# loryruta/gl-radix-sort

Measured on AMD Instinct MI355X. Metric: Mkeys/s sorting 2^28 uint32 key+val; % HBM roofline; 1/2/4/8 GPU, higher is better.
Workload: dtype u32; 1 GPU; 2^28 uint32 key + uint32 val pairs, uniform-random full-range keys, vals=iota, in-place stable radix sort, 1x MI355X; pairs_per_gpu=268435456, key_distribution=uniform, parallelism=single, device=AMD Radeon Graphics (gfx950:sramecc+:xnack-), 256 CUs, 288.0 GiB, device 0

## Files before the change

gl-radix-sort_amd/csrc/glu_hip.hip:

```cpp
#include <hip/hip_runtime.h>

#include <algorithm>
#include <cstdio>
#include <cstdlib>
#include <cstring>
#include <mutex>
#include <strings.h>
#include <vector>

#include "glu_host.hpp"
#include "glu_sort_driver.hpp"
#include "glu_sort_launch.hpp"
#include "radix_sort_kernels.hpp"
#include "radix_pair_passes.hpp"
#include "radix_lds_plan.hpp"

using namespace glu_hip;
using namespace glu_hip::host;

glu_status glu_hip::host::sort_prepare(glu_radix_sort_s* s, size_t count, size_t key_size, bool with_vals, bool may_place)
{
    if (count <= 1) return GLU_OK;
    const bool grows = s->keys.size < count * key_size || (with_vals && s->vals.size < count * sizeof(uint32_t));
    if (grows && !s->tuning)
// ... 208 lines not shown
    int cur = 0;
    uint32_t pass = 0;
    for (; pass < num_passes; pass++)
    {
        const uint32_t shift = passes[pass].shift, bits = passes[pass].bits, xform = passes[pass].xform;
        if (planned)
        {
            PlanArgs pa;
            pa.plan = (PassPlan*) s->plan.ptr;
            pa.pass = pass;
            pa.may_skip = xform == 0;
            if (key_xf == KEY_XF_NONE && !s->no_bit_shortcut) pa.flags = pass == 0 ? kPlanCollectBits : (pa.may_skip ? kPlanShortcut : 0u);
            pa.pair_role = passes[pass].pair_role;
            if (pa.pair_role == 1)
            {
                pa.shift2 = passes[pass + 1].shift;
                pa.bits2 = passes[pass + 1].bits;
            }
            s->cur_kind = finish_kpt && pass < 2 ? 1 : 0;
            pa.behind_attempt = finish_kpt && pass >= 2;
            s->cur_behind = pa.behind_attempt;
            if (finish_kpt && pass == 0)
            {
                pa.finish_geo_first = finish_kpt;
                pa.finish_geo_last = finish_last;
                pa.finish_first_ordinary = 2;
                pa.finish_num_ordinary = num_passes - 2;
                pa.finish_seq = s->feedback.finish_seq;
                pa.finish_top_bit = finish_top_bit;
                pa.finish_key_bits = end_bit;
                pa.finish_long_ok = finish_long_ok;
                pa.fork_side = fork;
            }
            pa.unitsum_side = fork && pass == 1 && pa.pair_role == 2 && bits == 8;
            if (finish_kpt && pass < 2 && s->last_narrow_offered) pa.narrow_keys = narrow_keys;
            GLU_TRY(dispatch_pass<KeyT>(s, kbuf[0], vbuf[0], kbuf[1], vbuf[1], count, shift, bits, nullptr,
                                        fork && pa.behind_attempt ? s->side : stream, xform, pa));
            if (finish_kpt && pass == 1)
            {
                if (fork) HIP_TRY(hipEventRecord(s->ev_fork2, stream));
                s->cur_kind = 2;
                s->cur_behind = false;
                s->mark(stream);
                s->mark(stream);
                const FinishMarks finish_marks{[](void* object, hipStream_t st) { ((glu_radix_sort_s*) object)->mark(st, true); }, s};
                const auto finish = vals ? (key_xf != KEY_XF_NONE ? launch_finish<KeyT, true, true> : launch_finish<KeyT, true, false>)
                                         : (key_xf != KEY_XF_NONE ? launch_finish<KeyT, false, true> : launch_finish<KeyT, false, false>);
                GLU_TRY(finish(kbuf[0], vbuf[0], kbuf[1], vbuf[1], (const uint32_t*) s->finish_starts.ptr, finish_kpt, finish_last, finish_expected,
                               finish_top_bit - 16u, pa.plan, 2u, key_xf, stream, s->finish_rank_bits, (uint32_t*) s->finish_crowded.ptr, finish_marks,
                               s->last_narrow_offered ? (const uint16_t*) narrow_keys : (const uint16_t*) nullptr));
                if (finish_long_ok && !fork)
                    GLU_TRY(launch_long_run_passes_any<KeyT>(s, kbuf[0], vbuf[0], kbuf[1], vbuf[1], count, key_xf, stream));
            }
        }
        else
        {
            GLU_TRY(dispatch_pass<KeyT>(s, kbuf[cur], vbuf[cur], kbuf[cur ^ 1], vbuf[cur ^ 1], count, shift, bits, nullptr,
                                        stream, xform));
            cur ^= 1;
        }
    }
    s->cur_behind = false;
    if (fork)
    {
        HIP_TRY(hipStreamWaitEvent(s->side, s->ev_fork2, 0));
        if (finish_long_ok) GLU_TRY(launch_long_run_passes_any<KeyT>(s, kbuf[0], vbuf[0], kbuf[1], vbuf[1], count, key_xf, s->side));
        HIP_TRY(side_join.join());
    }
    if (planned)
    {
        const dim3 grid((uint32_t) std::min<size_t>((count + 255) / 256, (size_t) g_dev.num_cus * 16));
        const auto finalize = vals ? radix_finalize_kernel<KeyT, true> : radix_finalize_kernel<KeyT, false>;
        hipLaunchKernelGGL(finalize, grid, dim3(256), 0, stream, kbuf[0], vbuf[0], (const KeyT*) kbuf[1], (const uint32_t*) vbuf[1],
                           (uint32_t) count, (const PassPlan*) s->plan.ptr, pass, finish_kpt ? 2u : 0u);
        HIP_TRY(hipGetLastError());
        return GLU_OK;
    }
    if (cur == 1)
    {
        HIP_TRY(hipMemcpyAsync(keys, kbuf[1], count * sizeof(KeyT), hipMemcpyDeviceToDevice, stream));
        if (vals) HIP_TRY(hipMemcpyAsync(vals, vbuf[1], count * sizeof(uint32_t), hipMemcpyDeviceToDevice, stream));
    }
    return GLU_OK;
}

template<typename KeyT>
glu_status glu_hip::host::sort_run(glu_radix_sort_s* s, KeyT* keys, uint32_t* vals, size_t count, size_t num_steps, hipStream_t stream,
                                   uint32_t key_xf)
{
    constexpr size_t kMaxSteps = sizeof(KeyT) * 2;
    const size_t steps = (num_steps == 0 || num_steps > kMaxSteps) ? kMaxSteps : num_steps;
    return sort_bits<KeyT>(s, keys, vals, count, 0u, (uint32_t) steps * 4, stream, key_xf);
}
template glu_status glu_hip::host::sort_bits<uint32_t>(glu_radix_sort_s*, uint32_t*, uint32_t*, size_t, uint32_t, uint32_t, hipStream_t, uint32_t);
template glu_status glu_hip::host::sort_bits<uint64_t>(glu_radix_sort_s*, uint64_t*, uint32_t*, size_t, uint32_t, uint32_t, hipStream_t, uint32_t);
template glu_status glu_hip::host::sort_run<uint32_t>(glu_radix_sort_s*, uint32_t*, uint32_t*, size_t, size_t, hipStream_t, uint32_t);
template glu_status glu_hip::host::sort_run<uint64_t>(glu_radix_sort_s*, uint64_t*, uint32_t*, size_t, size_t, hipStream_t, uint32_t);
// ... 423 lines not shown
```

gl-radix-sort_amd/csrc/glu_sort_driver.hpp:

```cpp
#pragma once
#include <vector>

#include "glu_sort_object.hpp"
#include "seg_plan.hpp"

namespace glu_hip
{
namespace host
{

glu_status sort_prepare(glu_radix_sort_s* s, size_t count, size_t key_size, bool with_vals = true, bool may_place = false);

template<typename KeyT>
glu_status sort_bits(glu_radix_sort_s* s, KeyT* keys, uint32_t* vals, size_t count, uint32_t first_bit, uint32_t end_bit,
                     hipStream_t stream, uint32_t key_xf = KEY_XF_NONE);
extern template glu_status sort_bits<uint32_t>(glu_radix_sort_s*, uint32_t*, uint32_t*, size_t, uint32_t, uint32_t, hipStream_t, uint32_t);
extern template glu_status sort_bits<uint64_t>(glu_radix_sort_s*, uint64_t*, uint32_t*, size_t, uint32_t, uint32_t, hipStream_t, uint32_t);

template<typename KeyT>
glu_status sort_run(glu_radix_sort_s* s, KeyT* keys, uint32_t* vals, size_t count, size_t num_steps, hipStream_t stream,
                    uint32_t key_xf = KEY_XF_NONE);
extern template glu_status sort_run<uint32_t>(glu_radix_sort_s*, uint32_t*, uint32_t*, size_t, size_t, hipStream_t, uint32_t);
extern template glu_status sort_run<uint64_t>(glu_radix_sort_s*, uint64_t*, uint32_t*, size_t, size_t, hipStream_t, uint32_t);

// ... 1 lines not shown


constexpr size_t kTuneMinKeyBytes = (size_t) 512 << 20;
glu_status tune_scratch_placement(glu_radix_sort_s* s, size_t count, size_t key_size);
glu_status place_pair_by_measurement(glu_radix_sort_s* s, size_t count, Scratch& keys, Scratch& vals);


constexpr size_t kSegMinCount = 1 << 16;
constexpr uint32_t kSegMaxSegments = 1u << 24;

struct SegPlan
{
    std::vector<SegPiece> pieces;
    std::vector<uint64_t> seg_start;
    uint32_t nseg = 0, passes = 0, bits = 0;
    size_t count = 0;
    bool by_copies = false;
    SegImage first, later;
    uint32_t max_subs_per_wg() const { return std::max(first.max_subs_per_wg, later.max_subs_per_wg); }
};

void seg_make_plan(glu_radix_sort_s* s, std::vector<SegPiece>&& pieces, uint32_t nseg, size_t count, uint32_t bits, bool aligned,
                   SegPlan& plan, uint64_t origin = 0);

bool seg_finish_choice_for(const glu_radix_sort_s* s, uint32_t passes, uint32_t bits, uint64_t nruns, uint64_t largest, uint32_t& geo,
                           uint32_t& split_log2);
bool seg_finish_choice(const glu_radix_sort_s* s, const SegPlan& plan, uint32_t& geo, uint32_t& split_log2);

glu_status seg_run_plan(glu_radix_sort_s* s, const SegPlan& plan, uint32_t* in_k, uint32_t* in_v, uint32_t* out_k, uint32_t* out_v,
                        hipStream_t stream);

glu_status read_seg_gate(const glu_radix_sort_s* s, bool& tried, uint32_t& longest);

template<typename KeyT>
glu_status launch_long_run_passes_any(glu_radix_sort_s* s, KeyT* a_k, uint32_t* a_v, KeyT* b_k, uint32_t* b_v, size_t count, uint32_t key_xf,
                                      hipStream_t stream);
extern template glu_status launch_long_run_passes_any<uint32_t>(glu_radix_sort_s*, uint32_t*, uint32_t*, uint32_t*, uint32_t*, size_t, uint32_t,
                                                                hipStream_t);
extern template glu_status launch_long_run_passes_any<uint64_t>(glu_radix_sort_s*, uint64_t*, uint32_t*, uint64_t*, uint32_t*, size_t, uint32_t,
                                                                hipStream_t);
}
}
```

gl-radix-sort_amd/csrc/glu_sort_object.hpp:

```cpp
#pragma once
#include <algorithm>
#include <chrono>
#include <cmath>
#include <cstdlib>
#include <cstring>
#include <mutex>
#include <string>
#include <vector>

#include "glu_batch_host.hpp"
#include "radix_sort_kernels.hpp"
#include "sort_call_plan.hpp"

namespace glu_hip
{
namespace host
{
constexpr int kMaxRadix = 256;
constexpr int kMaxBlocksPerCu = 4;

template<int THREADS_, int KPT_, int BLOCKS_PER_CU_, bool CARRY_>
struct Geometry
{
    static constexpr int THREADS = THREADS_, KPT = KPT_, BLOCKS_PER_CU = BLOCKS_PER_CU_, TILE = THREADS_ * KPT_;
// ... 79 lines not shown
    uint32_t last_seg_finish_capacity = 0, last_seg_finish_runs = 0, last_seg_finish_tile = 0, last_seg_finish_split = 0;
    uint32_t seg_split_max = 0;
    uint32_t seg_split_min = 0;
    uint32_t finish_rank_bits = 16;
    uint32_t seg_split_geo = 3;
    uint32_t seg_max_geo = 4;
    uint32_t digit_bits = 8;
    uint32_t max_blocks = 0;
    uint32_t reserved_cus = 0;
    bool force_small = false;
    bool no_single_block = false;
    bool no_fused_scan = false;
    bool no_plan = false;
    bool tune_scratch = true;
    bool tuning = false;
    uint32_t tuned_spacer_mib = 0, tuned_candidates = 0; double tuned_ms = 0, tuned_worst_ms = 0;
    bool no_lines = false;
    bool nt_stores = true;
    size_t nt_min_bytes = (size_t) 320 << 20;
    bool no_bit_shortcut = false;
    bool equal_shares = false;
    bool pairs = true;
    uint32_t last_pair_roles[kPlanMaxPasses] = {};
    size_t pair_min = 0;
    uint32_t pair_unit_div = 16;
    hipEvent_t after_histogram_event = nullptr;
    Scratch finish_lengths;
    Scratch finish_starts;
    Scratch finish_crowded;
    Scratch narrow_keys;
    bool narrow_handoff = true;
    bool last_narrow_offered = false;
    hipStream_t side = nullptr;
    hipEvent_t ev_fork = nullptr, ev_unit = nullptr, ev_fork2 = nullptr, ev_join = nullptr;
    bool fork_behind = true;
    bool side_forked = false;
    bool ensure_side()
    {
        if (side) return true;
        bool ok = true;
        for (hipEvent_t* e : {&ev_fork, &ev_unit, &ev_fork2, &ev_join})
            ok = ok && hipEventCreateWithFlags(e, hipEventDisableTiming) == hipSuccess;
        if (ok && hipStreamCreateWithFlags(&side, hipStreamNonBlocking) == hipSuccess) return true;
        for (hipEvent_t* e : {&ev_fork, &ev_unit, &ev_fork2, &ev_join})
        {
            if (*e) (void) hipEventDestroy(*e);
            *e = nullptr;
        }
        side = nullptr;
        return false;
    }
    bool lds_finish = true;
    bool long_runs = true;
    size_t finish_min = 0;
    uint32_t* finish_hint = nullptr;
    FinishFeedback feedback;
    bool device_top = true;
    bool last_device_top = false;
    uint32_t last_finish_top = 0;
    bool last_finish_attempted = false;
    bool last_finish_long_ok = false;
    uint32_t last_finish_capacity = 0;
    size_t large_min = 0;
    int profiling = 0;
    std::vector<hipEvent_t> events;
    size_t events_used = 0;
    std::vector<hipEvent_t> slots;
    hipEvent_t next_event()
    {
        if (events_used == events.size())
        {
            hipEvent_t e;
            if (hipEventCreate(&e) != hipSuccess) return nullptr;
            events.push_back(e);
        }
        return events[events_used++];
    }
// ... 1 lines not shown
    std::vector<uint32_t> pass_seqs;
    uint32_t cur_seq = 0;
    Scratch finish_outcomes;
    uint8_t cur_kind = 0;
    bool cur_behind = false;
    void mark(hipStream_t stream, bool around_data_kernel = false)
    {
        if (!profiling) return;
        if (slots.size() % 4 == 0) pass_kinds.push_back(cur_kind), pass_seqs.push_back(cur_seq), between_forms.push_back(nullptr);
        hipEvent_t e = nullptr;
        if (profiling == 1 || (around_data_kernel && !cur_behind))
            if ((e = next_event()) != nullptr) (void) hipEventRecord(e, stream);
        slots.push_back(e);
    }
    std::vector<hipEvent_t> between_forms;
    void mark_between_forms(hipStream_t stream)
    {
        if (!profiling || between_forms.empty() || (profiling != 1 && cur_behind)) return;
        hipEvent_t e = next_event();
        if (e && hipEventRecord(e, stream) == hipSuccess) between_forms.back() = e;
    }
    void clear_marks() { events_used = 0, slots.clear(), pass_kinds.clear(), pass_seqs.clear(), between_forms.clear(); }
    template<typename F>
    void for_each_scratch(F&& f)
    {
        for (Scratch* sc : {&keys, &vals, &table, &plan, &pair_t2, &pair_table, &pair_ranges, &pair_sub, &pair_wide, &seg_desc, &seg_zero, &batch_lists,
                            &long_image, &long_hdr, &long_bits, &seg_gate, &finish_lengths, &finish_starts, &finish_crowded, &finish_outcomes, &narrow_keys})
            f(*sc);
    }
    void release()
    {
        for_each_scratch([](Scratch& sc) { sc.release(); });
        if (finish_hint) (void) hipHostFree(finish_hint);
        for (hipEvent_t e : {ev_fork, ev_unit, ev_fork2, ev_join})
            if (e) (void) hipEventDestroy(e);
        if (side) (void) hipStreamDestroy(side);
        for (hipEvent_t e : events) (void) hipEventDestroy(e);
        for (SegStage& st : seg_stage)
        {
            if (st.host) (void) hipHostFree(st.host);
            if (st.copied) (void) hipEventDestroy(st.copied);
        }
    }
};

namespace glu_hip
{
namespace host
{
constexpr size_t kPairMinKeyBytes = (size_t) 1 << 28;
constexpr size_t finish_min_count(size_t key_size) { return key_size == 8 ? (size_t) 3 << 21 : (size_t) 7 << 22; }
constexpr size_t kPlanMinCount = (size_t) 1 << 22;

inline uint32_t usable_cus(const glu_radix_sort_s* s)
{
    return (uint32_t) std::max<int>(1, g_dev.num_cus - (int) s->reserved_cus);
}

struct PlanArgs
{
    PassPlan* plan = nullptr;
    uint32_t pass = 0;
    bool may_skip = false;
    int pair_role = 0;
    uint32_t shift2 = 0, bits2 = 0;
    uint32_t flags = 0;
    bool behind_attempt = false;
    uint32_t finish_geo_first = 0, finish_geo_last = 0;
    uint32_t finish_first_ordinary = 0, finish_num_ordinary = 0;
    uint32_t finish_seq = 0, finish_top_bit = 0, finish_key_bits = 0;
    bool finish_long_ok = false;
    bool fork_side = false;
    bool unitsum_side = false;
    uint16_t* narrow_keys = nullptr;
};

constexpr size_t kSmallResidentPerCU = 4;

template<typename KeyT, int BITS>
size_t large_tiles_from(const glu_radix_sort_s* s, bool vals, size_t large_tile)
{
    if (s->large_min) return s->large_min;
    size_t from = (size_t) g_dev.num_cus * large_tile * 3 / 2;
    const size_t small_tile = vals ? GeometryFor<KeyT, BITS, false, true>::TILE : GeometryFor<KeyT, BITS, false, false>::TILE;
    if (sizeof(KeyT) == 4 && vals) from = std::max<size_t>(from, (size_t) g_dev.num_cus * kSmallResidentPerCU * small_tile + 1);
    if (sizeof(KeyT) == 4 && !vals && BITS == 8) from = std::max<size_t>(from, (size_t) 1 << 25);
    return from;
}

template<typename KeyT, int BITS>
bool lines_applicable(const glu_radix_sort_s* s, const void* src_k, const void* src_v, const void* dst_k, const void* dst_v, size_t count)
{
    const bool vals = src_v != nullptr;
    const size_t lines_tile = vals ? LinesGeometry<KeyT, BITS, true>::TILE : LinesGeometry<KeyT, BITS, false>::TILE;
    const bool aligned = (((uintptr_t) src_k | (uintptr_t) src_v | (uintptr_t) dst_k | (uintptr_t) dst_v) & 15u) == 0;
    return aligned && !s->no_lines && !s->force_small && count >= lines_tile && count >= large_tiles_from<KeyT, BITS>(s, vals, lines_tile);
}

template<typename KeyT>
glu_status dispatch_pass(glu_radix_sort_s* s, const KeyT* src_k, const uint32_t* src_v, KeyT* dst_k, uint32_t* dst_v,
                         size_t count, uint32_t shift, uint32_t bits, uint32_t* histogram_out, hipStream_t stream,
                         uint32_t xform = 0, PlanArgs pa = PlanArgs());
extern template glu_status dispatch_pass<uint32_t>(glu_radix_sort_s*, const uint32_t*, const uint32_t*, uint32_t*, uint32_t*, size_t, uint32_t,
                                                   uint32_t, uint32_t*, hipStream_t, uint32_t, PlanArgs);
extern template glu_status dispatch_pass<uint64_t>(glu_radix_sort_s*, const uint64_t*, const uint32_t*, uint64_t*, uint32_t*, size_t, uint32_t,
                                                   uint32_t, uint32_t*, hipStream_t, uint32_t, PlanArgs);
// ... 3 lines not shown
```

gl-radix-sort_amd/csrc/glu_sort_passes.hpp:

```cpp
#pragma once
#include "glu_sort_object.hpp"
#include "radix_scatter_lines.hpp"
#include "radix_pair_passes.hpp"
#include "radix_lds_plan.hpp"

namespace glu_hip
{
namespace host
{
template<typename KeyT, int BITS, bool LARGE, bool XF, bool VALS>
glu_status launch_pass(glu_radix_sort_s* s, const KeyT* src_k, const uint32_t* src_v, KeyT* dst_k, uint32_t* dst_v,
                       size_t count, uint32_t shift, uint32_t bits, uint32_t* histogram_out, hipStream_t stream,
                       uint32_t xform = 0, PlanArgs pa = PlanArgs())
{
    using G = GeometryFor<KeyT, BITS, LARGE, VALS>;
    constexpr int RADIX = 1 << BITS;
    const uint32_t tiles = (uint32_t) ((count + G::TILE - 1) / G::TILE);
    uint64_t cap = (uint64_t) usable_cus(s) * G::BLOCKS_PER_CU;
    if (s->max_blocks) cap = std::min<uint64_t>(cap, s->max_blocks);
    const uint32_t nb = (uint32_t) std::max<uint64_t>(1, std::min<uint64_t>(tiles, cap));
    const uint32_t mask = (1u << bits) - 1;
    uint32_t* table = (uint32_t*) s->table.ptr;
    uint32_t* totals = table + (size_t) RADIX * nb;

    using Smem = ScatterSmem<KeyT, BITS, G::THREADS, G::KPT, G::CARRY, 1, VALS>;
    auto scatter = radix_scatter_kernel<KeyT, BITS, G::THREADS, G::KPT, G::CARRY, 0, false, G::BLOCKS_PER_CU * G::THREADS / 256, 1, false, false, XF, VALS>;
    auto scatter_fused = radix_scatter_kernel<KeyT, BITS, G::THREADS, G::KPT, G::CARRY, 0, false, G::BLOCKS_PER_CU * G::THREADS / 256, 1, false, false, XF, VALS, !LARGE>;
    constexpr uint32_t kRowSharers = G::THREADS / RADIX >= 1 ? G::THREADS / RADIX : 1;
    constexpr uint32_t kFusedLimit = kFusedScanMaxBlocks * (kRowSharers / 4 >= 1 ? kRowSharers / 4 : 1);
    const bool fused = !LARGE && nb <= kFusedLimit && !histogram_out && !s->no_fused_scan && !pa.plan;
    static std::once_flag lds_opt_in;
    static hipError_t lds_opt_in_result = hipSuccess;
    std::call_once(lds_opt_in, [&] {
        lds_opt_in_result = hipFuncSetAttribute((const void*) scatter, hipFuncAttributeMaxDynamicSharedMemorySize, (int) sizeof(Smem));
// ... 89 lines not shown
                auto count2_collect = radix_pair_count_kernel<KeyT, G::TILE, XF, !XF>;
                static std::once_flag count2_opt_in;
                static hipError_t count2_opt_in_result = hipSuccess;
                std::call_once(count2_opt_in, [&] {
                    count2_opt_in_result = hipFuncSetAttribute((const void*) count2_plain, hipFuncAttributeMaxDynamicSharedMemorySize, (int) sizeof(PairCountSmem));
                    if (count2_opt_in_result == hipSuccess)
                        count2_opt_in_result = hipFuncSetAttribute((const void*) count2_collect, hipFuncAttributeMaxDynamicSharedMemorySize, (int) sizeof(PairCountSmem));
                });
                HIP_TRY(count2_opt_in_result);
                auto count2 = (pa.flags & kPlanCollectBits) ? count2_collect : count2_plain;
                hipLaunchKernelGGL(count2, dim3(nb), dim3(1024), sizeof(PairCountSmem), stream, src_k, table, (uint32_t*) s->pair_t2.ptr,
                                   (uint32_t) count, shift, mask, pa.shift2, (1u << pa.bits2) - 1, tiles, xform, (const KeyT*) dst_k,
                                   pa.plan, pa.pass, pa.flags, share, pa.finish_geo_first ? (uint32_t*) s->pair_wide.ptr : (uint32_t*) nullptr);
            }
            else
            {
                auto count4_plain = radix_pair4_count_kernel<KeyT, G::TILE, false, false>;
                auto count4_collect = radix_pair4_count_kernel<KeyT, G::TILE, false, true>;
                hipLaunchKernelGGL((pa.flags & kPlanCollectBits) ? count4_collect : count4_plain,
                                   dim3(nb * kPairSub), dim3(256), 0, stream, src_k, sub_table, (uint32_t*) s->pair_t2.ptr, (uint32_t) count, shift, mask, pa.shift2,
                                   (1u << pa.bits2) - 1, tiles, xform, (const KeyT*) dst_k, pa.plan, pa.pass, pa.flags, share);
            }
            HIP_TRY(hipGetLastError());
        }
    }
    if (pa.pair_role == 2)
    {
        uint32_t* leader_table = table;
        table = (uint32_t*) s->pair_table.ptr;
        totals = table + (size_t) RADIX * nb;
        ranges = (const uint2*) s->pair_ranges.ptr;
        if constexpr (BITS == 8)
        {
            hipLaunchKernelGGL(radix_pair_unitsum_kernel, dim3(nb), dim3(1024), 0, pa.unitsum_side ? s->side : stream, (const uint32_t*) s->pair_t2.ptr,
                               (const uint32_t*) leader_table, (const uint32_t*) (leader_table + (size_t) RADIX * nb), table,
                               (uint2*) s->pair_ranges.ptr, (uint32_t) count, pa.plan, pa.pass, shift, mask, pa.flags);
            if (pa.unitsum_side)
            {
                HIP_TRY(hipEventRecord(s->ev_unit, s->side));
                HIP_TRY(hipStreamWaitEvent(stream, s->ev_unit, 0));
            }
        }
        else
            hipLaunchKernelGGL(radix_pair4_unitsum_kernel, dim3(nb), dim3(1024), 0, stream, (const uint32_t*) s->pair_t2.ptr,
                               (const uint32_t*) sub_table, (const uint32_t*) (leader_table + (size_t) RADIX * nb), table,
                               (uint2*) s->pair_ranges.ptr, (uint32_t) count, pa.plan, pa.pass, shift, mask, pa.flags);
        HIP_TRY(hipGetLastError());
    }
    if (pa.pair_role != 1)
    {
        auto count_plain = radix_count_kernel<KeyT, BITS, 1024, G::TILE, XF, false>;
        auto count_collect = radix_count_kernel<KeyT, BITS, 1024, G::TILE, XF, !XF>;
        hipLaunchKernelGGL((pa.flags & kPlanCollectBits) ? count_collect : count_plain, dim3(nb), dim3(1024), 0, stream, src_k, table,
                           (uint32_t) count, shift, mask, tiles, xform, (const KeyT*) dst_k, pa.plan, pa.pass, pa.pair_role == 2,
                           pa.flags, share);
        HIP_TRY(hipGetLastError());
    }
    s->mark(stream);
    if (BITS == 4 && pa.pair_role == 1)
    {
        hipLaunchKernelGGL((radix_row_scan_kernel<256>), dim3(RADIX), dim3(256), 0, stream, sub_table, totals, nb * kPairSub,
                           (uint32_t) count, pa.may_skip ? pa.plan : (PassPlan*) nullptr, pa.pass, 0u, pa.plan, table,
                           kPairSub);
    }
    else
    {
        hipLaunchKernelGGL((radix_row_scan_kernel<256>), dim3(RADIX), dim3(256), 0, stream, table, totals, nb, (uint32_t) count,
                           pa.may_skip ? pa.plan : (PassPlan*) nullptr, pa.pass,
                           pa.pair_role == 1 && BITS == 8
                               ? (s->pair_unit_div ? std::max<uint32_t>(1u, (uint32_t) (count / nb / s->pair_unit_div)) : 0xFFFFFFFFu)
                               : 0u,
                           pa.plan);
    }
    HIP_TRY(hipGetLastError());
    if (pa.finish_geo_first)
    {
        hipLaunchKernelGGL(radix_finish_lengths_kernel, dim3(kPairRadix), dim3(1024), 0, stream, (const uint32_t*) s->pair_t2.ptr, nb,
                           (uint32_t*) s->finish_lengths.ptr, (const PassPlan*) pa.plan, pa.pass, (const uint32_t*) s->pair_wide.ptr);
        HIP_TRY(hipGetLastError());
        const bool long_runs = pa.finish_long_ok && s->long_image.ptr;
        hipLaunchKernelGGL(radix_finish_plan_kernel, dim3(kFinishPlanBlocks), dim3(1024), 0, stream, (const uint32_t*) s->finish_lengths.ptr,
                           (uint32_t*) s->finish_starts.ptr, (uint32_t) count, pa.finish_geo_first, pa.finish_geo_last, pa.plan, pa.pass,
                           pa.finish_first_ordinary, pa.finish_num_ordinary, s->finish_hint, pa.finish_seq, pa.finish_top_bit,
                           pa.finish_key_bits, long_runs ? 1u : 0u, (uint32_t*) s->finish_crowded.ptr, (uint32_t*) s->finish_outcomes.ptr,
                           (uint32_t) (sizeof(KeyT) + (VALS ? sizeof(uint32_t) : 0)), pa.narrow_keys ? 1u : 0u);
        HIP_TRY(hipGetLastError());
        if (long_runs)
        {
            hipLaunchKernelGGL(radix_finish_long_runs_kernel, dim3(1), dim3(1024), 0, stream, (const uint32_t*) s->finish_starts.ptr,
                               (const PassPlan*) pa.plan, usable_cus(s) * kLongRunsSharesPerWg, (uint32_t*) s->long_image.ptr, (uint32_t*) s->long_hdr.ptr);
            HIP_TRY(hipGetLastError());
        }
        if (pa.fork_side)
        {
            HIP_TRY(hipEventRecord(s->ev_fork, stream));
            HIP_TRY(hipStreamWaitEvent(s->side, s->ev_fork, 0));
            s->side_forked = true;
        }
    }
    s->mark(stream, true);
    if (histogram_out)
    {
        HIP_TRY(hipMemcpyAsync(histogram_out, totals, ((size_t) 1 << bits) * sizeof(uint32_t), hipMemcpyDeviceToDevice,
                               stream));
        if (s->after_histogram_event) HIP_TRY(hipEventRecord(s->after_histogram_event, stream));
    }
    bool both_forms = false;
    if constexpr (sizeof(KeyT) == 4 && BITS == 8 && !XF && VALS)
    {
        both_forms = pa.narrow_keys && pa.pair_role == 2 && pa.plan;
        if (both_forms)
        {
            using NarrowSmem = LineSmem<KeyT, BITS, G::THREADS, G::KPT, VALS, true>;
            auto scatter_wide = nt ? lines_scatter_kernel<KeyT, BITS, XF, VALS, true, false, 1>() : lines_scatter_kernel<KeyT, BITS, XF, VALS, false, false, 1>();
            auto scatter_narrow = nt ? lines_scatter_kernel<KeyT, BITS, XF, VALS, true, false, 2>() : lines_scatter_kernel<KeyT, BITS, XF, VALS, false, false, 2>();
            static std::once_flag narrow_opt_in;
            static hipError_t narrow_opt_in_result = hipSuccess;
            std::call_once(narrow_opt_in, [&] {
                for (const void* k : {(const void*) lines_scatter_kernel<KeyT, BITS, XF, VALS, true, false, 1>(), (const void*) lines_scatter_kernel<KeyT, BITS, XF, VALS, false, false, 1>()})
                    if (narrow_opt_in_result == hipSuccess)
                        narrow_opt_in_result = hipFuncSetAttribute(k, hipFuncAttributeMaxDynamicSharedMemorySize, (int) sizeof(Smem));
                for (const void* k : {(const void*) lines_scatter_kernel<KeyT, BITS, XF, VALS, true, false, 2>(), (const void*) lines_scatter_kernel<KeyT, BITS, XF, VALS, false, false, 2>()})
                    if (narrow_opt_in_result == hipSuccess)
                        narrow_opt_in_result = hipFuncSetAttribute(k, hipFuncAttributeMaxDynamicSharedMemorySize, (int) sizeof(NarrowSmem));
            });
// ... 64 lines not shown
```

gl-radix-sort_amd/csrc/glu_sort_segments.hip:

```cpp
#include <hip/hip_runtime.h>

#include <algorithm>
#include <cstring>
#include <mutex>
#include <vector>

#include "glu_host.hpp"
#include "glu_sort_driver.hpp"
#include "glu_sort_launch.hpp"
#include "radix_sort_kernels.hpp"
#include "radix_scatter_lines.hpp"
#include "radix_seg_passes.hpp"
#include "radix_lds_plan.hpp"

using namespace glu_hip;
using namespace glu_hip::host;

namespace
{
template<typename KeyT, bool VALS, bool XF>
glu_status launch_long_run_passes(glu_radix_sort_s* s, KeyT* a_k, uint32_t* a_v, KeyT* b_k, uint32_t* b_v, size_t count, uint32_t key_xf,
                                  hipStream_t stream)
{
    using G = typename std::conditional<sizeof(KeyT) == 4 && VALS, SegLinesGeometry, LinesGeometry<KeyT, 8, VALS>>::type;
// ... 83 lines not shown
    {
        hipLaunchKernelGGL((radix_seg_runs_kernel<RADIX>), dim3(1), dim3(1024), 0, stream, (const uint32_t*) table, image + img.off_list,
                           image + img.off_start, img.nseg, runs_end, (uint32_t*) s->finish_starts.ptr, (uint32_t*) s->seg_gate.ptr);
        HIP_TRY(hipGetLastError());
    }
    s->mark(stream, true);
    hipLaunchKernelGGL(s->nt_stores ? scatter_nt : scatter_plain, dim3(img.nwg), dim3(G::THREADS), sizeof(Smem), stream, src_k, src_v,
                       dst_k, dst_v, (const uint32_t*) table, (const uint32_t*) nullptr, (uint32_t) count, shift, 255u, 0u,
                       (unsigned long long*) nullptr, 0u, (PassPlan*) nullptr, 0u, subs, 0u, image + img.off_first, gate, gate_cap, gate_mode, (const uint32_t*) nullptr,
                       (uint16_t*) nullptr);
    HIP_TRY(hipGetLastError());
    s->mark(stream, true);
    return GLU_OK;
}

glu_status read_pieces(const uint64_t* piece_begin, const uint64_t* piece_len, const uint32_t* piece_segment, size_t num_pieces,
                       uint32_t num_segments, const size_t* count, std::vector<SegPiece>& pieces, uint64_t& total)
{
    pieces.resize(num_pieces);
    total = 0;
    for (size_t i = 0; i < num_pieces; i++)
    {
        if (piece_segment[i] >= num_segments) return fail(GLU_ERROR_INVALID_ARGUMENT, "piece %zu names segment %u of %u", i, piece_segment[i], num_segments);
        if (count && (piece_begin[i] > *count || piece_len[i] > *count - piece_begin[i]))
            return fail(GLU_ERROR_INVALID_ARGUMENT, "piece %zu [%llu, +%llu) exceeds count %zu", i, (unsigned long long) piece_begin[i],
                        (unsigned long long) piece_len[i], *count);
        pieces[i] = SegPiece{piece_begin[i], piece_len[i], piece_segment[i]};
        total += piece_len[i];
    }
    return GLU_OK;
}
}

template<typename KeyT>
glu_status glu_hip::host::launch_long_run_passes_any(glu_radix_sort_s* s, KeyT* a_k, uint32_t* a_v, KeyT* b_k, uint32_t* b_v, size_t count,
                                                     uint32_t key_xf, hipStream_t stream)
{
    if (a_v) return key_xf != KEY_XF_NONE ? launch_long_run_passes<KeyT, true, true>(s, a_k, a_v, b_k, b_v, count, key_xf, stream)
                                          : launch_long_run_passes<KeyT, true, false>(s, a_k, a_v, b_k, b_v, count, key_xf, stream);
    return key_xf != KEY_XF_NONE ? launch_long_run_passes<KeyT, false, true>(s, a_k, nullptr, b_k, nullptr, count, key_xf, stream)
                                 : launch_long_run_passes<KeyT, false, false>(s, a_k, nullptr, b_k, nullptr, count, key_xf, stream);
}
template glu_status glu_hip::host::launch_long_run_passes_any<uint32_t>(glu_radix_sort_s*, uint32_t*, uint32_t*, uint32_t*, uint32_t*, size_t,
                                                                        uint32_t, hipStream_t);
template glu_status glu_hip::host::launch_long_run_passes_any<uint64_t>(glu_radix_sort_s*, uint64_t*, uint32_t*, uint64_t*, uint32_t*, size_t,
                                                                        uint32_t, hipStream_t);

void glu_hip::host::seg_make_plan(glu_radix_sort_s* s, std::vector<SegPiece>&& pieces, uint32_t nseg, size_t count, uint32_t bits,
                                  bool aligned, SegPlan& plan, uint64_t origin)
{
    plan.pieces = std::move(pieces);
    plan.nseg = nseg;
    plan.count = count;
    plan.bits = bits;
    plan.passes = bits / 8;
    seg_order_pieces(plan.pieces, nseg, origin, plan.seg_start);
    plan.by_copies = count < kSegMinCount || !aligned || plan.passes == 0;
    if (plan.by_copies) return;
    const uint32_t nwg = usable_cus(s);
    seg_build_image(plan.pieces.data(), plan.pieces.size(), nseg, plan.seg_start.data(), count, nwg, plan.first);
    if (plan.passes > 1)
    {
        std::vector<SegPiece> whole(nseg);
        for (uint32_t g = 0; g < nseg; g++) whole[g] = SegPiece{plan.seg_start[g], plan.seg_start[g + 1] - plan.seg_start[g], g};
        seg_build_image(whole.data(), whole.size(), nseg, plan.seg_start.data(), count, nwg, plan.later);
    }
// ... 211 lines not shown
```

gl-radix-sort_amd/csrc/radix_lds_plan.hpp:

```cpp
#pragma once

#include "radix_lds_finish.hpp"
#include "radix_pair_passes.hpp"

namespace glu_hip
{
constexpr uint32_t kSampleTopBlocks = 64;
template<typename KeyT>
__global__ __launch_bounds__(256) void radix_sample_top_kernel(const KeyT* __restrict__ keys, uint32_t n, uint32_t key_bits,
                                                               uint32_t floor_top, PassPlan* plan)
{
    typedef uint32_t u32x4_t __attribute__((ext_vector_type(4)));
    __shared__ uint32_t red[4][4];
    const uint32_t tid = threadIdx.x, lane = tid & 63, wave = tid >> 6;
    constexpr uint32_t W = sizeof(KeyT) / 4;
    const uint64_t nvec = (uint64_t) n * sizeof(KeyT) / 16;
    const uint32_t total = gridDim.x * 256u;
    const uint32_t samples = (uint32_t) (nvec < total ? nvec : total);
    const uint64_t stride = samples ? nvec / samples : 1;
    uint32_t o[2] = {0, 0}, no[2] = {0, 0};
    const uint32_t j = blockIdx.x * 256u + tid;
    if (j < samples)
    {
        const u32x4_t x = reinterpret_cast<const u32x4_t*>(keys)[(uint64_t) j * stride];
// ... 150 lines not shown
    {
        uint32_t a = ld(tid * PER), p = pos, g = seg;
        for (uint32_t j = 0; j < PER; j++)
        {
            const uint32_t e = ld(tid * PER + j + 1), l = e - a;
            if (l > cap)
            {
                image[lay.off_list + g] = sb;
                image[lay.off_start + g] = a;
                for (uint32_t w = p / share; w <= (p + l - 1) / share; w++)
                {
                    const uint32_t b0 = max(p, w * share), b1 = min(p + l, (w + 1) * share);
                    image[2 * sb] = a + (b0 - p);
                    image[2 * sb + 1] = a + (b1 - p);
                    if (b0 == w * share) image[lay.off_first + w] = sb;
                    sb++;
                }
                p += l;
                g++;
            }
            a = e;
        }
    }
    __syncthreads();
    if (tid == 0)
    {
        hdr[1] = nsb;
        image[lay.off_list + nseg] = nsb;
    }
    for (uint32_t w = tid; w <= nwg; w += 1024)
        if (image[lay.off_first + w] == 0xFFFFFFFFu) image[lay.off_first + w] = nsb;
}

static __global__ __launch_bounds__(1024) void radix_finish_lengths_kernel(const uint32_t* __restrict__ t2, uint32_t nb,
                                                                    uint32_t* __restrict__ lengths, const PassPlan* plan,
                                                                    uint32_t pass, const uint32_t* __restrict__ wide = nullptr)
{
    if (plan->off[pass] || plan->skip[pass] == kSkipWithoutCounting) return;
    __shared__ uint32_t part[8][kPairRadix];
    __shared__ uint32_t wide_list[1024], wide_n;
    const uint32_t tid = threadIdx.x, g = tid >> 7, q = tid & 127u, d = blockIdx.x;
    uint32_t lo = 0, hi = 0;
#pragma unroll 4
    for (uint32_t b = g; b < nb; b += 8)
    {
        const uint32_t w = t2[((size_t) d * nb + b) * kPairRowWords + q];
        lo += w & 0xFFFFu;
        hi += w >> 16;
    }
    part[g][2 * q] = lo;
    part[g][2 * q + 1] = hi;
    if (tid == 0) wide_n = 0;
    __syncthreads();
    if (wide && tid < nb)
    {
        const uint32_t* hdr = wide + (size_t) tid * kPairWideStride;
        const uint32_t nw = hdr[0] <= kPairWideRows ? hdr[0] : 0u;
        for (uint32_t k = 0; k < nw; k++)
            if (hdr[1 + k] == d) wide_list[atomicAdd(&wide_n, 1u)] = (tid << 8) | k;
    }
    __syncthreads();
    if (tid < kPairRadix)
    {
        uint32_t c = 0;
#pragma unroll
        for (int k = 0; k < 8; k++) c += part[k][tid];
        for (uint32_t i = 0; i < wide_n; i++)
        {
            const uint32_t bk = wide_list[i];
            c += wide[(size_t) (bk >> 8) * kPairWideStride + 16 + (bk & 255u) * kPairRadix + tid] << 16;
        }
        lengths[tid * kPairRadix + d] = c;
    }
}

static __global__ __launch_bounds__(1024) void radix_finish_plan_kernel(const uint32_t* __restrict__ lengths, uint32_t* starts,
                                                                 uint32_t n, uint32_t geo_first, uint32_t geo_last, PassPlan* plan,
                                                                 uint32_t pass,
                                                                 uint32_t first_ordinary, uint32_t num_ordinary,
                                                                 uint32_t* hint, uint32_t attempt, uint32_t top_bit,
                                                                 uint32_t key_bits, uint32_t long_ok, uint32_t* crowded_lists,
                                                                 uint32_t* outcomes = nullptr, uint32_t pair_bytes = 8,
                                                                 uint32_t narrow_ok = 0)
{
    __shared__ uint32_t tmp[3][16];
    __shared__ uint32_t over_tmp[2][kFinishGeometries][16];
    const uint32_t tid = threadIdx.x, lane = tid & 63, wave = tid >> 6, b = blockIdx.x;
    const bool tables = !(plan->off[pass] || plan->skip[pass] == kSkipWithoutCounting);
    uint32_t before = 0, all = 0, longest = 0, mine = 0;
    uint32_t over_len[kFinishGeometries] = {}, over_cnt[kFinishGeometries] = {};
    if (tables)
    {
#pragma unroll
        for (uint32_t j = 0; j < kFinishPlanBlocks; j++)
        {
            const uint32_t v = lengths[j * 1024u + tid];
            all += v;
            before += j < b ? v : 0u;
            longest = max(longest, v);
            mine = j == b ? v : mine;
            if (long_ok && b == 0)
            {
#pragma unroll
                for (uint32_t g = 0; g < kFinishGeometries; g++)
                {
                    const bool over = v > finish_geometry_capacity(g + 1);
// ... 72 lines not shown
    starts[b * 1024u + tid] = before + excl;
    if (b == 0 && tid == 0) starts[kFinishRuns] = n;
    if (b == 0 && crowded_lists && tid < kCrowdedLists) crowded_lists[tid * kCrowdedCountStride] = 0u;
    if (b == 0 && tid == 0)
    {
        plan->finish = accept ? geo : 0u;
        plan->finish_longest = tables ? longest : 0xFFFFFFFFu;
        if (outcomes) outcomes[attempt & 255u] = (attempt << 3) | (accept ? geo : 0u);
        {
            const uint32_t low_bits = top_bit - 16u;
            const uint64_t low_mask = low_bits >= 64u ? ~0ull : (1ull << low_bits) - 1ull;
            const uint32_t to_order = plan->bits_valid ? (uint32_t) __popcll(varying & low_mask) : low_bits;
            plan->finish_rounds = to_order < 9u ? 1u : 0u;
            const bool narrow = accept && narrow_ok != 0u && to_order >= 9u && longest <= finish_geometry_capacity(geo) && low_bits <= 16u;
            const uint32_t common_hi = plan->bits_valid && top_bit < 32u ? plan->bits_or[0] & ~((1u << top_bit) - 1u) : 0u;
            plan->narrow = narrow ? 1u | (common_hi & kPlanNarrowHiMask) : 0u;
            if (outcomes) outcomes[256u + (attempt & 255u)] = (attempt << 1) | (narrow ? 1u : 0u);
        }
        if (hint)
        {
            if (plan->bits_valid)
            {
                __hip_atomic_store(hint + 1, (uint32_t) varying, __ATOMIC_RELAXED, __HIP_MEMORY_SCOPE_SYSTEM);
                __hip_atomic_store(hint + 2, (uint32_t) (varying >> 32), __ATOMIC_RELAXED, __HIP_MEMORY_SCOPE_SYSTEM);
                __hip_atomic_store(hint + 3, attempt, __ATOMIC_RELAXED, __HIP_MEMORY_SCOPE_SYSTEM);
            }
            __hip_atomic_store(hint + 4, top_bit, __ATOMIC_RELAXED, __HIP_MEMORY_SCOPE_SYSTEM);
            __hip_atomic_store(hint, (attempt << 3) | (accept ? geo : 0u), __ATOMIC_RELEASE, __HIP_MEMORY_SCOPE_SYSTEM);
        }
        if (!accept)
        {
            plan->skip[pass] = kSkipWithoutCounting;
            plan->off[pass + 1] = 1;
            plan->flip[pass + 1] = plan->flip[pass + 2] = pass > 0 ? plan->flip[pass] : 0u;
        }
    }
    if (b == 0 && accept && tid < num_ordinary) plan->off[first_ordinary + tid] = 1;
}


static __global__ __launch_bounds__(1024) void radix_finish_long_runs_kernel(const uint32_t* __restrict__ starts, const PassPlan* plan,
                                                                      uint32_t nwg, uint32_t* __restrict__ image, uint32_t* __restrict__ hdr)
{
    __shared__ uint32_t wsum[2][16];
    finish_list_long_runs(starts, plan->finish, plan->finish_longest, nwg, image, hdr, wsum);
}

}
```

gl-radix-sort_amd/csrc/radix_pair_passes.hpp:

```cpp
#pragma once

#include "radix_sort_kernels.hpp"

namespace glu_hip
{
constexpr uint32_t kPairRadix = 256;
constexpr uint32_t kPairRowWords = kPairRadix / 2;
constexpr uint32_t kPairMaxRunUnits = 2048;

__device__ __forceinline__ uint32_t pair_word(uint32_t d, uint32_t e) { return d * kPairRowWords + ((e >> 1) ^ (d & 63u)); }

struct PairCountSmem
{
    static constexpr int WAVES = 16;
    uint32_t hist1[WAVES][kPairRadix];
    uint32_t hist2[kPairRadix * kPairRowWords];
};

constexpr uint32_t kPairWideRows = 14;
constexpr uint32_t kPairWideStride = 16 + kPairWideRows * 256;

template<typename KeyT, int TILE, bool XF = false, bool COLLECT = false>
__global__ __launch_bounds__(1024) void radix_pair_count_kernel(const KeyT* __restrict__ keys_a, uint32_t* __restrict__ table,
                                                                uint32_t* __restrict__ t2, uint32_t n, uint32_t shift,
// ... 217 lines not shown
    for (int side = 0; side < 2; side++)
    {
        const uint32_t P = (uint32_t) ((uint64_t) n * (w + side) / nb);
        if (w + side == nb)
        {
            edge[side] = (uint32_t) RADIX * row_len;
            edge_start[side] = n;
            continue;
        }
        if (tid < 2) found[tid] = 0;
        __syncthreads();
        if (tid < (uint32_t) RADIX && base[tid] < P) atomicAdd(&found[0], 1u);
        __syncthreads();
        const uint32_t below = found[0];
        if (below == 0)
        {
            edge[side] = 0;
            edge_start[side] = 0;
            continue;
        }
        const uint32_t ds = below - 1;
        uint32_t mine = 0;
        for (uint32_t i = tid; i < row_len; i += blockDim.x)
            if (base[ds] + scanned[(size_t) ds * row_len + i] < P) mine++;
        if (mine) atomicAdd(&found[1], mine);
        __syncthreads();
        const uint32_t in_row = found[1];
        edge[side] = ds * row_len + in_row;
        edge_start[side] = in_row < row_len ? base[ds] + scanned[(size_t) ds * row_len + in_row] : base[ds + 1];
        __syncthreads();
    }
}

static __global__ __launch_bounds__(1024) void radix_pair_unitsum_kernel(const uint32_t* __restrict__ t2,
                                                                  const uint32_t* __restrict__ table_l,
                                                                  const uint32_t* __restrict__ totals_l,
                                                                  uint32_t* __restrict__ table_f, uint2* __restrict__ ranges,
                                                                  uint32_t n, PassPlan* plan, uint32_t pass,
                                                                  uint32_t shift = 0, uint32_t mask = 0, uint32_t plan_flags = 0)
{
    if (plan->off[pass])
    {
        if (blockIdx.x == 0 && threadIdx.x == 0) plan->skip[pass] = kSkipWithoutCounting;
        return;
    }
    if (plan->pair_fallback[pass]) return;
    shift -= plan->shift_down[pass];
    if ((plan_flags & kPlanShortcut) && plan_digit_is_constant(plan, shift, mask))
    {
        if (blockIdx.x == 0 && threadIdx.x == 0) plan->skip[pass] = kSkipWithoutCounting;
        return;
    }
    __shared__ uint32_t base[kPairRadix + 1];
    __shared__ uint32_t tmp[16];
    __shared__ uint32_t found[2];
    __shared__ uint32_t part[32][kPairRadix];
    const uint32_t tid = threadIdx.x;
    const uint32_t nb = gridDim.x, w = blockIdx.x;
    if (w == 0 && tid == 0) plan->skip[pass] = 0;
    pair_unit_bases<kPairRadix>(totals_l, n, base, tmp);
    uint32_t edge[2], edge_start[2];
    pair_find_run<kPairRadix>(table_l, nb, base, found, n, w, nb, edge, edge_start);

    if (edge[1] - edge[0] > kPairMaxRunUnits)
    {
        if (tid == 0) plan->pair_fallback[pass] = 1;
        return;
    }
    const uint32_t g = tid >> 5, q = tid & 31u;
    uint32_t acc[8] = {0, 0, 0, 0, 0, 0, 0, 0};
    const uint4* rows = reinterpret_cast<const uint4*>(t2);
#pragma unroll 4
    for (uint32_t u = edge[0] + g; u < edge[1]; u += 32)
    {
        const uint4 v = rows[(size_t) u * (kPairRowWords / 4) + q];
        acc[0] += v.x & 0xFFFFu, acc[1] += v.x >> 16, acc[2] += v.y & 0xFFFFu, acc[3] += v.y >> 16;
        acc[4] += v.z & 0xFFFFu, acc[5] += v.z >> 16, acc[6] += v.w & 0xFFFFu, acc[7] += v.w >> 16;
    }
#pragma unroll
    for (int k = 0; k < 8; k++) part[g][8 * q + k] = acc[k];
    __syncthreads();
    if (tid < kPairRadix)
    {
        uint32_t c = 0;
#pragma unroll
        for (int k = 0; k < 32; k++) c += part[k][tid];
        table_f[(size_t) tid * nb + w] = c;
    }
    if (tid == 0) ranges[w] = make_uint2(edge_start[0], edge_start[1]);
}

constexpr uint32_t kPairSub = 16;
constexpr uint32_t kPair4Radix = 16;

template<typename KeyT, int TILE, bool XF = false, bool COLLECT = false>
__global__ __launch_bounds__(256) void radix_pair4_count_kernel(const KeyT* __restrict__ keys_a, uint32_t* __restrict__ table_sub,
                                                                uint32_t* __restrict__ t2, uint32_t n, uint32_t shift,
                                                                uint32_t mask, uint32_t shift2, uint32_t mask2,
                                                                uint32_t tiles_total, uint32_t xform, const KeyT* keys_b,
                                                                PassPlan* plan, uint32_t pass, uint32_t plan_flags = 0,
                                                                uint32_t share = 0)
{
    constexpr int THREADS = 256;
    constexpr int WAVES = THREADS / kWave;
    __shared__ uint32_t hist[WAVES][256];
    const uint32_t tid = threadIdx.x, lane = tid & 63, wave = tid >> 6;
    const uint32_t nb = gridDim.x / kPairSub, b = blockIdx.x / kPairSub, j = blockIdx.x % kPairSub;
    const KeyT* __restrict__ keys = keys_a;
    if (plan)
    {
        if ((plan_flags & kPlanShortcut) && plan_digit_is_constant(plan, shift, mask))
        {
            if (blockIdx.x == 0 && tid == 0)
            {
                plan->skip[pass] = kSkipWithoutCounting;
                plan->pair_fallback[pass + 1] = 1;
            }
            return;
        }
        if (pass > 0 && plan->flip[pass]) keys = keys_b;
        if (blockIdx.x == 0 && tid == 0)
        {
// ... 145 lines not shown
```

Before: 75450 Mkeys/s.

## Fuse pair unitsum into finish-lengths kernel and move long-runs planning to side stream

The separate unitsum kernel for the second pair pass, which previously could run on the side stream with an event handshake, is now computed by extra blocks appended to the finish-lengths kernel. This saves a launch and the cross-stream event sync. The long-runs planning kernel is also moved onto the side stream when forking, so it overlaps with the main stream. The unitsum logic is factored into a shared device function. The fused launch makes the lengths kernel grid larger and adds skip-flag propagation, which introduces ordering subtleties around plan flags.

After: 75510 Mkeys/s, median of 2. No clear change (+0.1%).

```diff
diff --git a/gl-radix-sort_amd/csrc/glu_hip.hip b/gl-radix-sort_amd/csrc/glu_hip.hip
--- a/gl-radix-sort_amd/csrc/glu_hip.hip
+++ b/gl-radix-sort_amd/csrc/glu_hip.hip
@@ -264,7 +264,11 @@
                 pa.finish_long_ok = finish_long_ok;
                 pa.fork_side = fork;
             }
-            pa.unitsum_side = fork && pass == 1 && pa.pair_role == 2 && bits == 8;
+            if (finish_kpt && pass < 2 && passes[0].pair_role == 1 && passes[1].pair_role == 2 && passes[0].bits == 8 && passes[1].bits == 8)
+            {
+                pa.units_with_lengths = true;
+                if (key_xf == KEY_XF_NONE && !s->no_bit_shortcut && passes[1].xform == 0) pa.flags2 = kPlanShortcut;
+            }
             if (finish_kpt && pass < 2 && s->last_narrow_offered) pa.narrow_keys = narrow_keys;
             GLU_TRY(dispatch_pass<KeyT>(s, kbuf[0], vbuf[0], kbuf[1], vbuf[1], count, shift, bits, nullptr,
                                         fork && pa.behind_attempt ? s->side : stream, xform, pa));
@@ -295,6 +299,7 @@
     s->cur_behind = false;
     if (fork)
     {
+        if (finish_long_ok) GLU_TRY(launch_finish_long_runs(s, (const PassPlan*) s->plan.ptr, s->side));
         HIP_TRY(hipStreamWaitEvent(s->side, s->ev_fork2, 0));
         if (finish_long_ok) GLU_TRY(launch_long_run_passes_any<KeyT>(s, kbuf[0], vbuf[0], kbuf[1], vbuf[1], count, key_xf, s->side));
         HIP_TRY(side_join.join());
diff --git a/gl-radix-sort_amd/csrc/glu_sort_driver.hpp b/gl-radix-sort_amd/csrc/glu_sort_driver.hpp
--- a/gl-radix-sort_amd/csrc/glu_sort_driver.hpp
+++ b/gl-radix-sort_amd/csrc/glu_sort_driver.hpp
@@ -57,6 +57,8 @@
 
 glu_status read_seg_gate(const glu_radix_sort_s* s, bool& tried, uint32_t& longest);
 
+glu_status launch_finish_long_runs(glu_radix_sort_s* s, const PassPlan* plan, hipStream_t stream);
+
 template<typename KeyT>
 glu_status launch_long_run_passes_any(glu_radix_sort_s* s, KeyT* a_k, uint32_t* a_v, KeyT* b_k, uint32_t* b_v, size_t count, uint32_t key_xf,
                                       hipStream_t stream);
diff --git a/gl-radix-sort_amd/csrc/glu_sort_object.hpp b/gl-radix-sort_amd/csrc/glu_sort_object.hpp
--- a/gl-radix-sort_amd/csrc/glu_sort_object.hpp
+++ b/gl-radix-sort_amd/csrc/glu_sort_object.hpp
@@ -135,17 +135,17 @@
     bool narrow_handoff = true;
     bool last_narrow_offered = false;
     hipStream_t side = nullptr;
-    hipEvent_t ev_fork = nullptr, ev_unit = nullptr, ev_fork2 = nullptr, ev_join = nullptr;
+    hipEvent_t ev_fork = nullptr, ev_fork2 = nullptr, ev_join = nullptr;
     bool fork_behind = true;
     bool side_forked = false;
     bool ensure_side()
     {
         if (side) return true;
         bool ok = true;
-        for (hipEvent_t* e : {&ev_fork, &ev_unit, &ev_fork2, &ev_join})
+        for (hipEvent_t* e : {&ev_fork, &ev_fork2, &ev_join})
             ok = ok && hipEventCreateWithFlags(e, hipEventDisableTiming) == hipSuccess;
         if (ok && hipStreamCreateWithFlags(&side, hipStreamNonBlocking) == hipSuccess) return true;
-        for (hipEvent_t* e : {&ev_fork, &ev_unit, &ev_fork2, &ev_join})
+        for (hipEvent_t* e : {&ev_fork, &ev_fork2, &ev_join})
         {
             if (*e) (void) hipEventDestroy(*e);
             *e = nullptr;
@@ -213,7 +213,7 @@
     {
         for_each_scratch([](Scratch& sc) { sc.release(); });
         if (finish_hint) (void) hipHostFree(finish_hint);
-        for (hipEvent_t e : {ev_fork, ev_unit, ev_fork2, ev_join})
+        for (hipEvent_t e : {ev_fork, ev_fork2, ev_join})
             if (e) (void) hipEventDestroy(e);
         if (side) (void) hipStreamDestroy(side);
         for (hipEvent_t e : events) (void) hipEventDestroy(e);
@@ -252,7 +252,8 @@
     uint32_t finish_seq = 0, finish_top_bit = 0, finish_key_bits = 0;
     bool finish_long_ok = false;
     bool fork_side = false;
-    bool unitsum_side = false;
+    bool units_with_lengths = false;
+    uint32_t flags2 = 0;
     uint16_t* narrow_keys = nullptr;
 };
 
diff --git a/gl-radix-sort_amd/csrc/glu_sort_passes.hpp b/gl-radix-sort_amd/csrc/glu_sort_passes.hpp
--- a/gl-radix-sort_amd/csrc/glu_sort_passes.hpp
+++ b/gl-radix-sort_amd/csrc/glu_sort_passes.hpp
@@ -1,5 +1,6 @@
 #pragma once
 #include "glu_sort_object.hpp"
+#include "glu_sort_driver.hpp"
 #include "radix_scatter_lines.hpp"
 #include "radix_pair_passes.hpp"
 #include "radix_lds_plan.hpp"
@@ -155,14 +156,10 @@
         ranges = (const uint2*) s->pair_ranges.ptr;
         if constexpr (BITS == 8)
         {
-            hipLaunchKernelGGL(radix_pair_unitsum_kernel, dim3(nb), dim3(1024), 0, pa.unitsum_side ? s->side : stream, (const uint32_t*) s->pair_t2.ptr,
-                               (const uint32_t*) leader_table, (const uint32_t*) (leader_table + (size_t) RADIX * nb), table,
-                               (uint2*) s->pair_ranges.ptr, (uint32_t) count, pa.plan, pa.pass, shift, mask, pa.flags);
-            if (pa.unitsum_side)
-            {
-                HIP_TRY(hipEventRecord(s->ev_unit, s->side));
-                HIP_TRY(hipStreamWaitEvent(stream, s->ev_unit, 0));
-            }
+            if (!pa.units_with_lengths)
+                hipLaunchKernelGGL(radix_pair_unitsum_kernel, dim3(nb), dim3(1024), 0, stream, (const uint32_t*) s->pair_t2.ptr,
+                                   (const uint32_t*) leader_table, (const uint32_t*) (leader_table + (size_t) RADIX * nb), table,
+                                   (uint2*) s->pair_ranges.ptr, (uint32_t) count, pa.plan, pa.pass, shift, mask, pa.flags);
         }
         else
             hipLaunchKernelGGL(radix_pair4_unitsum_kernel, dim3(nb), dim3(1024), 0, stream, (const uint32_t*) s->pair_t2.ptr,
@@ -198,8 +195,10 @@
     HIP_TRY(hipGetLastError());
     if (pa.finish_geo_first)
     {
-        hipLaunchKernelGGL(radix_finish_lengths_kernel, dim3(kPairRadix), dim3(1024), 0, stream, (const uint32_t*) s->pair_t2.ptr, nb,
-                           (uint32_t*) s->finish_lengths.ptr, (const PassPlan*) pa.plan, pa.pass, (const uint32_t*) s->pair_wide.ptr);
+        hipLaunchKernelGGL(radix_finish_lengths_units_kernel, dim3(kPairRadix + (pa.units_with_lengths ? nb : 0u)), dim3(1024), 0, stream,
+                           (const uint32_t*) s->pair_t2.ptr, nb, (uint32_t*) s->finish_lengths.ptr, pa.plan, pa.pass,
+                           (const uint32_t*) s->pair_wide.ptr, (const uint32_t*) table, (const uint32_t*) totals, (uint32_t*) s->pair_table.ptr,
+                           (uint2*) s->pair_ranges.ptr, (uint32_t) count, pa.shift2, (1u << pa.bits2) - 1, pa.flags2);
         HIP_TRY(hipGetLastError());
         const bool long_runs = pa.finish_long_ok && s->long_image.ptr;
         hipLaunchKernelGGL(radix_finish_plan_kernel, dim3(kFinishPlanBlocks), dim3(1024), 0, stream, (const uint32_t*) s->finish_lengths.ptr,
@@ -208,12 +207,7 @@
                            pa.finish_key_bits, long_runs ? 1u : 0u, (uint32_t*) s->finish_crowded.ptr, (uint32_t*) s->finish_outcomes.ptr,
                            (uint32_t) (sizeof(KeyT) + (VALS ? sizeof(uint32_t) : 0)), pa.narrow_keys ? 1u : 0u);
         HIP_TRY(hipGetLastError());
-        if (long_runs)
-        {
-            hipLaunchKernelGGL(radix_finish_long_runs_kernel, dim3(1), dim3(1024), 0, stream, (const uint32_t*) s->finish_starts.ptr,
-                               (const PassPlan*) pa.plan, usable_cus(s) * kLongRunsSharesPerWg, (uint32_t*) s->long_image.ptr, (uint32_t*) s->long_hdr.ptr);
-            HIP_TRY(hipGetLastError());
-        }
+        if (long_runs && !pa.fork_side) GLU_TRY(launch_finish_long_runs(s, pa.plan, stream));
         if (pa.fork_side)
         {
             HIP_TRY(hipEventRecord(s->ev_fork, stream));
diff --git a/gl-radix-sort_amd/csrc/glu_sort_segments.hip b/gl-radix-sort_amd/csrc/glu_sort_segments.hip
--- a/gl-radix-sort_amd/csrc/glu_sort_segments.hip
+++ b/gl-radix-sort_amd/csrc/glu_sort_segments.hip
@@ -139,6 +139,14 @@
 }
 }
 
+glu_status glu_hip::host::launch_finish_long_runs(glu_radix_sort_s* s, const PassPlan* plan, hipStream_t stream)
+{
+    hipLaunchKernelGGL(radix_finish_long_runs_kernel, dim3(1), dim3(1024), 0, stream, (const uint32_t*) s->finish_starts.ptr, plan,
+                       usable_cus(s) * kLongRunsSharesPerWg, (uint32_t*) s->long_image.ptr, (uint32_t*) s->long_hdr.ptr);
+    HIP_TRY(hipGetLastError());
+    return GLU_OK;
+}
+
 template<typename KeyT>
 glu_status glu_hip::host::launch_long_run_passes_any(glu_radix_sort_s* s, KeyT* a_k, uint32_t* a_v, KeyT* b_k, uint32_t* b_v, size_t count,
                                                      uint32_t key_xf, hipStream_t stream)
diff --git a/gl-radix-sort_amd/csrc/radix_lds_plan.hpp b/gl-radix-sort_amd/csrc/radix_lds_plan.hpp
--- a/gl-radix-sort_amd/csrc/radix_lds_plan.hpp
+++ b/gl-radix-sort_amd/csrc/radix_lds_plan.hpp
@@ -206,14 +206,13 @@
         if (image[lay.off_first + w] == 0xFFFFFFFFu) image[lay.off_first + w] = nsb;
 }
 
-static __global__ __launch_bounds__(1024) void radix_finish_lengths_kernel(const uint32_t* __restrict__ t2, uint32_t nb,
-                                                                    uint32_t* __restrict__ lengths, const PassPlan* plan,
-                                                                    uint32_t pass, const uint32_t* __restrict__ wide = nullptr)
+__device__ __forceinline__ void finish_lengths_block(const uint32_t* __restrict__ t2, uint32_t nb, uint32_t* __restrict__ lengths,
+                                                     PassPlan* plan, uint32_t pass, const uint32_t* __restrict__ wide, uint32_t d)
 {
     if (plan->off[pass] || plan->skip[pass] == kSkipWithoutCounting) return;
     __shared__ uint32_t part[8][kPairRadix];
     __shared__ uint32_t wide_list[1024], wide_n;
-    const uint32_t tid = threadIdx.x, g = tid >> 7, q = tid & 127u, d = blockIdx.x;
+    const uint32_t tid = threadIdx.x, g = tid >> 7, q = tid & 127u;
     uint32_t lo = 0, hi = 0;
 #pragma unroll 4
     for (uint32_t b = g; b < nb; b += 8)
@@ -246,6 +245,26 @@
         }
         lengths[tid * kPairRadix + d] = c;
     }
+}
+
+static __global__ __launch_bounds__(1024) void radix_finish_lengths_units_kernel(const uint32_t* __restrict__ t2, uint32_t nb,
+                                                                          uint32_t* __restrict__ lengths, PassPlan* plan, uint32_t pass,
+                                                                          const uint32_t* __restrict__ wide,
+                                                                          const uint32_t* __restrict__ table_l, const uint32_t* __restrict__ totals_l,
+                                                                          uint32_t* __restrict__ table_f, uint2* __restrict__ ranges, uint32_t n,
+                                                                          uint32_t shift_f, uint32_t mask_f, uint32_t flags_f)
+{
+    if (blockIdx.x < kPairRadix)
+    {
+        finish_lengths_block(t2, nb, lengths, plan, pass, wide, blockIdx.x);
+        return;
+    }
+    if (plan->off[pass] || plan->skip[pass] == kSkipWithoutCounting)
+    {
+        if (blockIdx.x == kPairRadix && threadIdx.x == 0) plan->skip[pass + 1] = kSkipWithoutCounting;
+        return;
+    }
+    pair_unitsum_block(t2, table_l, totals_l, table_f, ranges, n, plan, pass + 1, shift_f, mask_f, flags_f, blockIdx.x - kPairRadix, nb);
 }
 
 static __global__ __launch_bounds__(1024) void radix_finish_plan_kernel(const uint32_t* __restrict__ lengths, uint32_t* starts,
@@ -384,6 +403,7 @@
         {
             plan->skip[pass] = kSkipWithoutCounting;
             plan->off[pass + 1] = 1;
+            plan->skip[pass + 1] = kSkipWithoutCounting;
             plan->flip[pass + 1] = plan->flip[pass + 2] = pass > 0 ? plan->flip[pass] : 0u;
         }
     }
diff --git a/gl-radix-sort_amd/csrc/radix_pair_passes.hpp b/gl-radix-sort_amd/csrc/radix_pair_passes.hpp
--- a/gl-radix-sort_amd/csrc/radix_pair_passes.hpp
+++ b/gl-radix-sort_amd/csrc/radix_pair_passes.hpp
@@ -273,6 +273,61 @@
     }
 }
 
+__device__ __forceinline__ void pair_unitsum_block(const uint32_t* __restrict__ t2, const uint32_t* __restrict__ table_l,
+                                                   const uint32_t* __restrict__ totals_l, uint32_t* __restrict__ table_f,
+                                                   uint2* __restrict__ ranges, uint32_t n, PassPlan* plan, uint32_t pass, uint32_t shift,
+                                                   uint32_t mask, uint32_t plan_flags, uint32_t w, uint32_t nb)
+{
+    if (plan->off[pass])
+    {
+        if (w == 0 && threadIdx.x == 0) plan->skip[pass] = kSkipWithoutCounting;
+        return;
+    }
+    if (plan->pair_fallback[pass]) return;
+    shift -= plan->shift_down[pass];
+    if ((plan_flags & kPlanShortcut) && plan_digit_is_constant(plan, shift, mask))
+    {
+        if (w == 0 && threadIdx.x == 0) plan->skip[pass] = kSkipWithoutCounting;
+        return;
+    }
+    __shared__ uint32_t base[kPairRadix + 1];
+    __shared__ uint32_t tmp[16];
+    __shared__ uint32_t found[2];
+    __shared__ uint32_t part[32][kPairRadix];
+    const uint32_t tid = threadIdx.x;
+    if (w == 0 && tid == 0) plan->skip[pass] = 0;
+    pair_unit_bases<kPairRadix>(totals_l, n, base, tmp);
+    uint32_t edge[2], edge_start[2];
+    pair_find_run<kPairRadix>(table_l, nb, base, found, n, w, nb, edge, edge_start);
+
+    if (edge[1] - edge[0] > kPairMaxRunUnits)
+    {
+        if (tid == 0) plan->pair_fallback[pass] = 1;
+        return;
+    }
+    const uint32_t g = tid >> 5, q = tid & 31u;
+    uint32_t acc[8] = {0, 0, 0, 0, 0, 0, 0, 0};
+    const uint4* rows = reinterpret_cast<const uint4*>(t2);
+#pragma unroll 4
+    for (uint32_t u = edge[0] + g; u < edge[1]; u += 32)
+    {
+        const uint4 v = rows[(size_t) u * (kPairRowWords / 4) + q];
+        acc[0] += v.x & 0xFFFFu, acc[1] += v.x >> 16, acc[2] += v.y & 0xFFFFu, acc[3] += v.y >> 16;
+        acc[4] += v.z & 0xFFFFu, acc[5] += v.z >> 16, acc[6] += v.w & 0xFFFFu, acc[7] += v.w >> 16;
+    }
+#pragma unroll
+    for (int k = 0; k < 8; k++) part[g][8 * q + k] = acc[k];
+    __syncthreads();
+    if (tid < kPairRadix)
+    {
+        uint32_t c = 0;
+#pragma unroll
+        for (int k = 0; k < 32; k++) c += part[k][tid];
+        table_f[(size_t) tid * nb + w] = c;
+    }
+    if (tid == 0) ranges[w] = make_uint2(edge_start[0], edge_start[1]);
+}
+
 static __global__ __launch_bounds__(1024) void radix_pair_unitsum_kernel(const uint32_t* __restrict__ t2,
                                                                   const uint32_t* __restrict__ table_l,
                                                                   const uint32_t* __restrict__ totals_l,
@@ -280,55 +335,7 @@
                                                                   uint32_t n, PassPlan* plan, uint32_t pass,
                                                                   uint32_t shift = 0, uint32_t mask = 0, uint32_t plan_flags = 0)
 {
-    if (plan->off[pass])
-    {
-        if (blockIdx.x == 0 && threadIdx.x == 0) plan->skip[pass] = kSkipWithoutCounting;
-        return;
-    }
-    if (plan->pair_fallback[pass]) return;
-    shift -= plan->shift_down[pass];
-    if ((plan_flags & kPlanShortcut) && plan_digit_is_constant(plan, shift, mask))
-    {
-        if (blockIdx.x == 0 && threadIdx.x == 0) plan->skip[pass] = kSkipWithoutCounting;
-        return;
-    }
-    __shared__ uint32_t base[kPairRadix + 1];
-    __shared__ uint32_t tmp[16];
-    __shared__ uint32_t found[2];
-    __shared__ uint32_t part[32][kPairRadix];
-    const uint32_t tid = threadIdx.x;
-    const uint32_t nb = gridDim.x, w = blockIdx.x;
-    if (w == 0 && tid == 0) plan->skip[pass] = 0;
-    pair_unit_bases<kPairRadix>(totals_l, n, base, tmp);
-    uint32_t edge[2], edge_start[2];
-    pair_find_run<kPairRadix>(table_l, nb, base, found, n, w, nb, edge, edge_start);
-
-    if (edge[1] - edge[0] > kPairMaxRunUnits)
-    {
-        if (tid == 0) plan->pair_fallback[pass] = 1;
-        return;
-    }
-    const uint32_t g = tid >> 5, q = tid & 31u;
-    uint32_t acc[8] = {0, 0, 0, 0, 0, 0, 0, 0};
-    const uint4* rows = reinterpret_cast<const uint4*>(t2);
-#pragma unroll 4
-    for (uint32_t u = edge[0] + g; u < edge[1]; u += 32)
-    {
-        const uint4 v = rows[(size_t) u * (kPairRowWords / 4) + q];
-        acc[0] += v.x & 0xFFFFu, acc[1] += v.x >> 16, acc[2] += v.y & 0xFFFFu, acc[3] += v.y >> 16;
-        acc[4] += v.z & 0xFFFFu, acc[5] += v.z >> 16, acc[6] += v.w & 0xFFFFu, acc[7] += v.w >> 16;
-    }
-#pragma unroll
-    for (int k = 0; k < 8; k++) part[g][8 * q + k] = acc[k];
-    __syncthreads();
-    if (tid < kPairRadix)
-    {
-        uint32_t c = 0;
-#pragma unroll
-        for (int k = 0; k < 32; k++) c += part[k][tid];
-        table_f[(size_t) tid * nb + w] = c;
-    }
-    if (tid == 0) ranges[w] = make_uint2(edge_start[0], edge_start[1]);
+    pair_unitsum_block(t2, table_l, totals_l, table_f, ranges, n, plan, pass, shift, mask, plan_flags, blockIdx.x, gridDim.x);
 }
 
 constexpr uint32_t kPairSub = 16;
```
